# TankMermaid/GraphAligner

Hardware: AMD Instinct MI355X
Metric: aligned Gbp/sec (whole node), 10kb ONT reads vs chr-scale GFA (higher is better)
Workload: dtype u64

## Files before the change

__graft_entry__.py:

```python
import os
import subprocess
import sys

ROOT = os.path.dirname(os.path.abspath(__file__))
CSRC = os.path.join(ROOT, "graphaligner_amd", "csrc")
PRODUCT_SO = os.path.join(ROOT, "graphaligner_amd", "libgraphaligner_amd.so")
HIPCC = os.environ.get("HIPCC", "/opt/rocm/bin/hipcc")


def _run(cmd):
    print("+", " ".join(cmd), file=sys.stderr, flush=True)
    subprocess.check_call(cmd, stdout=sys.stderr)


def _stale(target, sources):
    if not os.path.exists(target):
        return True
    t = os.path.getmtime(target)
    return any(os.path.getmtime(s) > t for s in sources)


def build_stamped():
    obj = os.path.join(ROOT, "build")
    os.makedirs(obj, exist_ok=True)
# ... 11 lines not shown

def _hipcc_device(flags, out):
    import json
    import re
    cmd = [HIPCC, "--offload-arch=gfx950", "-O3", "-std=c++17", "-fPIC", "-Wno-unused-value", "-Rpass-analysis=kernel-resource-usage"] + flags + \
          ["-c", os.path.join(CSRC, "ga_device.hip"), "-o", out]
    print("+", " ".join(cmd), file=sys.stderr, flush=True)
    p = subprocess.run(cmd, stdout=subprocess.PIPE, stderr=subprocess.PIPE, text=True)
    table, cur = {}, None
    rest = []
    for line in p.stderr.splitlines():
        m = re.search(r"remark:\s+(.*?) \[-Rpass-analysis=kernel-resource-usage\]", line)
        if not m:
            rest.append(line)
            continue
        key, _, val = m.group(1).partition(":")
        key, val = key.strip(), val.strip()
        if key == "Function Name":
            name = subprocess.run(["c++filt", val], stdout=subprocess.PIPE, text=True).stdout.strip() or val
            name = re.sub(r"^void |\(anonymous namespace\)::|\(.*$", "", name)
            cur = table.setdefault(name, {})
        elif cur is not None:
            cur[key] = val
    sys.stderr.write("\n".join(l for l in rest if "warning" in l or "error" in l) + ("\n" if rest else ""))
    if p.returncode != 0:
        sys.stderr.write(p.stderr)
        raise subprocess.CalledProcessError(p.returncode, cmd)
    os.makedirs(os.path.dirname(RESOURCES_JSON), exist_ok=True)
    json.dump(table, open(RESOURCES_JSON, "w"), indent=1)
    print("%-52s %5s %5s %8s %7s %7s %5s %7s" % ("kernel", "VGPR", "AGPR", "scratch", "vSpill", "sSpill", "occ", "LDS"), file=sys.stderr)
    for name, r in table.items():
        print("%-52s %5s %5s %8s %7s %7s %5s %7s" % (name, r.get("VGPRs"), r.get("AGPRs"), r.get("ScratchSize [bytes/lane]"), r.get("VGPRs Spill"), r.get("SGPRs Spill"),
                                                     r.get("Occupancy [waves/SIMD]"), r.get("LDS Size [bytes/block]")), file=sys.stderr)
    no_scratch = ("ga_lanes_kernel", "ga_wide_kernel", "ga_wide_sparse_kernel", "ga_plan_", "ga_eq_words_", "ga_ops_", "ga_pileup_")
    bad = [n for n, r in table.items() if n.startswith(no_scratch) and int(r.get("ScratchSize [bytes/lane]", "0")) != 0]
    bad += [n for n, r in table.items() if n.startswith(("ga_lanes_kernel<10, 64>", "ga_plan_", "ga_eq_words_", "ga_ops_", "ga_pileup_")) and int(r.get("VGPRs Spill", "0")) != 0]
    if bad:
        raise RuntimeError("kernel resource check failed (private segment in a lanes = reads, state-in-HBM, plan or match-word kernel / vector "
                           "spills in <10,64>, a plan or a match-word kernel): %s" % ", ".join(bad))
    return table


def build_product(force=False):
    srcs = [os.path.join(CSRC, f) for f in os.listdir(CSRC)] + [os.path.join(ROOT, "include", "graphaligner_amd.h")]
    if not force and (os.environ.get("GA_SKIP_BUILD") == "1" or not _stale(PRODUCT_SO, srcs)) and os.path.exists(PRODUCT_SO):
        return
    obj = os.path.join(ROOT, "build")
    os.makedirs(obj, exist_ok=True)
    _run(["g++", "-std=c++17", "-O2", "-g", "-fPIC", "-ffp-contract=off", "-Wall", "-c", os.path.join(CSRC, "ga_host.cpp"), "-o", os.path.join(obj, "ga_host.o")])
    _run(["g++", "-std=c++17", "-O2", "-g", "-fPIC", "-Wall", "-c", os.path.join(CSRC, "ga_vgio.cpp"), "-o", os.path.join(obj, "ga_vgio.o")])
    _run(["g++", "-std=c++17", "-O2", "-g", "-fPIC", "-Wall", "-c", os.path.join(CSRC, "ga_seed_host.cpp"), "-o", os.path.join(obj, "ga_seed_host.o")])
    _hipcc_device(["-DGA_WAVES_EU=%s" % os.environ.get("GA_WAVES_EU", "6")], os.path.join(obj, "ga_device.o"))
    _run([HIPCC, "--offload-arch=gfx950", "-shared", "-pthread", "-o", PRODUCT_SO, os.path.join(obj, "ga_host.o"), os.path.join(obj, "ga_vgio.o"), os.path.join(obj, "ga_seed_host.o"), os.path.join(obj, "ga_device.o"), "-lz"])


def build():
    build_product()
    _run(["make", "-s", "-C", os.path.join(ROOT, "oracle")])
    _run(["make", "-s", "-C", os.path.join(ROOT, "tests", "emul")])
    _run(["make", "-s", "-C", os.path.join(ROOT, "tests", "emul"), "-f", "pileup.mk"])
    _run(["make", "-s", "-C", os.path.join(ROOT, "tests", "native")])
    sys.path.insert(0, ROOT)
    import graphaligner_amd
    from graphaligner_amd import binding
    binding.load()


# ... 21 lines not shown
```

graphaligner_amd/csrc/ga_device.hip:

```cpp
#include <hip/hip_runtime.h>

#include <algorithm>
#include <cstdio>
#include <cstdlib>
#include <cstring>
#include <memory>
#include <mutex>
#include <vector>

#include "../../include/graphaligner_amd.h"
#include "ga_backend.h"
#include "ga_kernel.h"
#include "ga_ladder.h"
#include "ga_lanes.h"
#include "ga_seed_dev.h"
#include "ga_plan.h"
#include "ga_ops.h"
#include "ga_pileup.h"

namespace {

#define HIP_OK(call) do { hipError_t e_ = (call); if (e_ != hipSuccess) { fprintf(stderr, "graphaligner_amd: %s failed: %s\n", #call, hipGetErrorString(e_)); return GA_E_DEVICE; } } while (0)

struct SlotLayout
// ... 77 lines not shown
		uint32_t job = L.job_list ? L.job_list[k] : k;
		gak::run_job<kWideNodes, true, false>(L, ws, slot, job);
		__syncthreads();
	}
}

__global__ void __launch_bounds__(64) ga_wide_sparse_kernel(GaLaunch L)
{
	const SlotLayout lay = slotLayout(L.cap_cols, L.max_slices, L.arena_words, L.trace_cap, L.sparse_bw, sizeof(gak::WaveState<kWideNodes>), kWideNodes);
	uint8_t* base = L.scratch + (uint64_t)blockIdx.x * L.slot_bytes;
	gak::WaveState<kWideNodes>& ws = *(gak::WaveState<kWideNodes>*)(base + lay.state);
	gak::Slot slot;
	slot.end_prev = (uint32_t*)(base + lay.endPrev);
	slot.end_cur = (uint32_t*)(base + lay.endCur);
	slot.slice_off = (uint32_t*)(base + lay.sliceOff);
	slot.arena = (uint32_t*)(base + lay.arena);
	slot.trace = base + lay.trace;
	slot.slice_flags = base + lay.flags;
	slot.ckpt = (uint32_t*)(base + lay.ckpt);
	slot.below_off = (uint32_t*)(base + lay.belowOff);
	slot.sparse = base + lay.sparse;
	slot.ovr = (uint32_t*)(base + lay.ovr);
	slot.sparse_max_bw = L.sparse_bw;
	while (true)
	{
		uint32_t k = gaw::wave_atomic_add(L.next_job, 1u);
		if (k >= L.n_jobs) break;
		uint32_t job = L.job_list ? L.job_list[k] : k;
		gak::run_job<kWideNodes, true, true>(L, ws, slot, job);
		__syncthreads();
	}
}

template <int N, int LW>
__global__ void __launch_bounds__(64) __attribute__((amdgpu_waves_per_eu(1, 2))) ga_lanes_kernel(gal::GaLanesLaunch L)
{
	using namespace gal;
	__shared__ uint32_t lds[Lay<N>::WORDS * LW + LW * kStageWords64 * 2 + 128];
	const int lane = (int)threadIdx.x;
	const WaveLayout lay = wave_layout<N>(L.cap_cols, L.cap_rows, L.max_slices, L.cap_moves, LW);
	uint8_t* base = L.scratch + (uint64_t)blockIdx.x * L.wave_bytes;
	while (true)
	{
		const uint32_t grp = gaw::wave_atomic_add(L.next_group, 1u);
		const uint64_t first = (uint64_t)grp * L.lanes_per_wave;
		if (first >= L.n_jobs) break;
		const bool hasJob = lane < (int)L.lanes_per_wave && lane < LW && first + (uint32_t)lane < L.n_jobs;
		const uint32_t jobIndex = hasJob ? (L.job_list ? L.job_list[first + (uint32_t)lane] : (uint32_t)(first + (uint32_t)lane)) : 0u;
		LaneMem m;
		m.lane = lane < LW ? lane : 0;
		m.tid = lane;
		m.flushPart = (uint32_t)lane % 12u; m.flushLane = (uint32_t)lane / 12u;
		m.ls = LW;
		m.lds.base = lds + (lane < LW ? lane : 0);
		m.lds.lw = LW;
		m.stage = (uint64_t*)(lds + Lay<N>::WORDS * LW);
		m.laneBlocks = lds + Lay<N>::WORDS * LW + LW * kStageWords64 * 2;
		m.usedChunks = 12u * (L.lanes_per_wave < (uint32_t)LW ? L.lanes_per_wave : (uint32_t)LW);
		m.endPrev = (uint32_t*)(base + lay.endA) + m.lane;
		m.endCur = (uint32_t*)(base + lay.endB) + m.lane;
		m.hdr = (uint32_t*)(base + lay.hdr) + m.lane;
		m.snodes = (uint32_t*)(base + lay.snodes) + m.lane;
		m.moves = (uint32_t*)(base + lay.moves) + m.lane;
		m.arena = base + lay.arena;
		LaneState st;
#if GA_STAMPS == 3
		const uint64_t wall0 = wall_clock64(), cyc0 = gaw::stamp();
#endif
		uint64_t tA = gaw::stamp(), tB, acc[4] = {0, 0, 0, 0};
#define GAL_LAP(i) do { tB = gaw::stamp(); acc[i] += tB - tA; tA = tB; } while (0)
		lane_begin<N>(L, m, st, jobIndex, hasJob);
		uint32_t blockTop = 0;
		for (uint32_t slice = 0; ; slice++)
		{
			lane_band<N>(L, m, st, slice);
			GAL_LAP(0);
			if (!__ballot(st.live)) break;
			fill_slice<N, 8, LW>(L.graph, m, st, slice, st.live, blockTop, L.cap_rows, L.cap_cols);
			GAL_LAP(1);
			lane_end_slice<N>(L, m, st, slice);
			GAL_LAP(2);
		}
		lane_finish<N>(L, m, st, hasJob);
		GAL_LAP(3);
#undef GAL_LAP
#ifdef GA_STAMPS
		if (hasJob && lane == 0) { GaJobOut* o = L.outs + st.job; o->stamps[1] = acc[0]; o->stamps[4] = acc[1]; o->stamps[0] = acc[2]; o->stamps[5] = acc[3]; o->stamps[2] = st.laps[0]; o->stamps[3] = st.laps[1]; o->stamps[6] = st.laps[2]; o->stamps[7] = st.laps[7];
#if GA_STAMPS == 4
			o->stamps[6] = acc[0]; o->stamps[7] = acc[1];
			for (int i = 0; i < 5; i++) o->stamps[i] = st.blaps[i];
#endif
#if GA_STAMPS == 3
			o->stamps[0] = wall0; o->stamps[1] = wall_clock64(); o->stamps[4] = gaw::stamp() - cyc0;
#endif
#if GA_STAMPS == 2
			o->stamps[0] = st.laps[4]; o->stamps[1] = st.laps[5]; o->stamps[4] = st.laps[6];
#endif
		}
#endif
		__syncthreads();
	}
}

__device__ __forceinline__ void eq_words_body(const uint8_t* __restrict__ seq, const GaEqFill* __restrict__ fills, uint32_t nFills, const uint8_t* __restrict__ lut,
                                              uint32_t padCode, uint64_t* __restrict__ eq, uint8_t* __restrict__ flags, uint8_t* __restrict__ rows)
{
	__shared__ uint8_t t[512];
	const uint32_t lane = threadIdx.x;
	for (uint32_t i = lane; i < 512; i += 64) t[i] = lut[i];
	__syncthreads();
	for (uint32_t fi = blockIdx.x; fi < nFills; fi += gridDim.x)
	{
		const GaEqFill f = fills[fi];
		const uint8_t* s = seq + f.seq_off;
		bool bad = false;
		for (uint32_t r0 = 0; r0 < f.padded; r0 += 64)
		{
			const uint32_t k = r0 + lane;
			uint32_t code = padCode;
			if (k < f.n) code = f.backward ? t[256 + s[f.n - 1 - k]] : t[s[f.pos + k]];
			rows[f.eq_slice * 64 + k] = (uint8_t)code;
			const uint64_t e0 = __ballot(code & 1u), e1 = __ballot(code & 2u), e2 = __ballot(code & 4u), e3 = __ballot(code & 8u);
			const uint64_t inv = __ballot(code & GA_ROW_INVALID);
			const uint32_t last = (uint32_t)__builtin_amdgcn_readlane((int)code, 63);
			const uint64_t meta = (uint64_t)((last >> 4) & 7u) | (inv ? 8u : 0u);
			if (lane < 5) eq[(f.eq_slice + r0 / 64) * 5 + lane] = lane == 0 ? e0 : lane == 1 ? e1 : lane == 2 ? e2 : lane == 3 ? e3 : meta;
			bad = bad || inv != 0;
		}
		if (lane == 0) flags[fi] = bad ? 1 : 0;
	}
}
__global__ void __launch_bounds__(64) ga_eq_words_kernel(const uint8_t* __restrict__ seq, const GaEqFill* __restrict__ fills, uint32_t nFills, const uint8_t* __restrict__ lut,
                                                         uint32_t padCode, uint64_t* __restrict__ eq, uint8_t* __restrict__ flags, uint8_t* __restrict__ rows)
{
// ... 604 lines not shown
		uint32_t maxRows = 0;
		for (uint32_t i : list) maxRows = std::max(maxRows, jobs[i].n_rows);
		P.max_slices = std::max<uint32_t>(maxRows / 64, 1);
		P.cap_cols = std::min<uint32_t>(N * 256u, 0xff00u);
		P.cap_moves = maxRows * 2 + 1024;
		const uint32_t ldsBytes = gal::Lay<N>::WORDS * LW * 4 + LW * gal::kStageWords64 * 8 + 512;
		const uint32_t wavesPerCu = std::max<uint32_t>(1, std::min<uint32_t>(8, 163840u / ldsBytes));
		auto layoutFor = [&](uint32_t lanes) {
			P.cap_rows = (uint32_t)std::min<uint64_t>(((uint64_t)P.max_slices * rowsPerSlice * lanes + 64 + 7u) & ~7ull, 0x7ffffff0ull);
			return gal::wave_layout<N>(P.cap_cols, P.cap_rows, P.max_slices, P.cap_moves, LW);
		};
		gal::WaveLayout lay = layoutFor(LW);
		const uint64_t fit = scratchBudget() / std::max<uint64_t>(lay.bytes, 1);
		uint64_t slotsHere = std::max<uint64_t>(1, std::min<uint64_t>((uint64_t)g->cus * wavesPerCu, std::max<uint64_t>(fit, 64)));
		if (knobs.waveSlots) slotsHere = std::min<uint64_t>(slotsHere, knobs.waveSlots);
		uint32_t lanesPer = LW;
		if (knobs.spread > 1) lanesPer = (uint32_t)std::min<int>(LW, knobs.spread);
		else if (knobs.spread && list.size() * 10 < slotsHere * LW * 6)
			lanesPer = (uint32_t)std::min<uint64_t>(LW, std::max<uint64_t>(8, (list.size() + slotsHere - 1) / slotsHere));
		P.lanes_per_wave = lanesPer;
		lay = layoutFor(lanesPer);
		P.wave_bytes = lay.bytes;
		const uint64_t groups = (list.size() + lanesPer - 1) / lanesPer;
		const uint32_t waves = (uint32_t)std::max<uint64_t>(1, std::min<uint64_t>(slotsHere, groups));
		bool fromPool = false;
		uint8_t* scratch = takeScratch((size_t)waves * lay.bytes, fromPool);
		if (!scratch) return 0;
		P.scratch = scratch;
		int rc = uploadList(list);
		if (!rc)
		{
			hipMemsetAsync(L.next_job, 0, 16, stream);
			hipEventRecord(evA, stream);
			hipLaunchKernelGGL((ga_lanes_kernel<N, LW>), dim3(waves), dim3(64), 0, stream, P);
			float ms = 0;
			rc = afterPass(ms);
			if (first) { st.main_ms = ms; st.main_variant = N * 1000 + 80 + (LW == 64 ? 0 : 1); st.slots = waves; st.waves_per_cu = wavesPerCu; st.scratch_bytes = (uint64_t)waves * lay.bytes; }
			if (knobs.debugPasses) fprintf(stderr, "graphaligner_amd: lanes pass <%d,%d>: %zu jobs on %u waves of %u lanes (%.1f GB scratch), %.2f ms\n", N, LW, list.size(), waves, lanesPer, waves * (double)lay.bytes / 1e9, ms);
#if GA_STAMPS == 3
			{
				uint64_t lo = ~0ull, hi = 0, n = 0; double life = 0, cyc = 0, lateStart = 0;
				for (auto& o : outs) if (o.stamps[1]) { lo = std::min(lo, o.stamps[0]); hi = std::max(hi, o.stamps[1]); }
				for (auto& o : outs) if (o.stamps[1]) { n++; life += (double)(o.stamps[1] - o.stamps[0]); cyc += (double)o.stamps[4]; lateStart = std::max(lateStart, (double)(o.stamps[0] - lo)); }
				{
					std::vector<std::pair<double, uint64_t>> lives;
					for (auto& o : outs) if (o.stamps[1]) lives.push_back({(double)(o.stamps[1] - o.stamps[0]) / 1e5, o.stamps[7]});
					std::sort(lives.begin(), lives.end());
					auto at = [&](double q) { return lives[(size_t)(q * (lives.size() - 1))]; };
					if (!lives.empty()) fprintf(stderr, "graphaligner_amd: wave life ms p10 %.2f p50 %.2f p90 %.2f p99 %.2f max %.2f; traceback rounds of the p10 / p50 / p99 / max wave: %llu / %llu / %llu / %llu, fast iterations %llu / %llu / %llu / %llu\n",
						at(0.1).first, at(0.5).first, at(0.9).first, at(0.99).first, at(1.0).first,
						(unsigned long long)(at(0.1).second & 0xffffffffu), (unsigned long long)(at(0.5).second & 0xffffffffu), (unsigned long long)(at(0.99).second & 0xffffffffu), (unsigned long long)(at(1.0).second & 0xffffffffu),
						(unsigned long long)(at(0.1).second >> 32), (unsigned long long)(at(0.5).second >> 32), (unsigned long long)(at(0.99).second >> 32), (unsigned long long)(at(1.0).second >> 32));
				}
				if (n) fprintf(stderr, "graphaligner_amd: %llu waves: first start to last end %.3f ms, mean wave life %.3f ms = %.1f M shader cycles (%.2f GHz), latest start %.3f ms after the first\n",
				               (unsigned long long)n, (hi - lo) / 1e5, life / n / 1e5, cyc / n / 1e6, cyc / life / 10.0, lateStart / 1e5);
			}
#endif
		}
		if (fromPool) g->givePool();
		return rc;
	}

	struct WaveKernel
	{
		void (*kernel)(GaLaunch);
		int maxN;
		bool general;
// ... 404 lines not shown
```

graphaligner_amd/csrc/ga_lanes.h:

```cpp
#pragma once
#include <stdint.h>

#include "ga_types.h"

namespace gal {

#ifdef GA_EMULATE
#define GAL_FN inline
#else
#define GAL_FN __device__ __forceinline__
#endif

#if defined(GA_STAMPS) && !defined(GA_EMULATE)
GAL_FN uint64_t lap_clock() { return __builtin_readcyclecounter(); }
#else
GAL_FN uint64_t lap_clock() { return 0; }
#endif

constexpr int W = 64;
constexpr int INF = 0x3fffffff;
constexpr uint32_t kCutoff = 200000;
constexpr int kRecBytes = 24;
constexpr int kHdrWords = 8;
constexpr uint32_t kNone = 0xffu;
// ... 1035 lines not shown
	{
		const unsigned long long prev = atomicCAS((unsigned long long*)top, seen, seen + (unsigned long long)bytes);
		if (prev == seen) return seen;
		seen = prev;
	}
	return ~0ull;
}
GAL_FN bool claim_for_wave(uint64_t* top, uint64_t cap, uint64_t bytes, uint64_t& at)
{
	const uint64_t active = __ballot(1);
	const int lane = (int)(threadIdx.x & 63);
	uint64_t before = 0, total = 0;
	for (uint64_t m = active; m; m &= m - 1)
	{
		const int src = __builtin_ctzll(m);
		const uint64_t b = ((uint64_t)(uint32_t)__shfl((int)(uint32_t)(bytes >> 32), src, 64) << 32) | (uint32_t)__shfl((int)(uint32_t)bytes, src, 64);
		if (src < lane) before += b;
		total += b;
	}
	const int leader = __builtin_ctzll(active);
	uint64_t base = ~0ull;
	if (lane == leader) base = claim_cas(top, cap, total);
	base = ((uint64_t)(uint32_t)__shfl((int)(uint32_t)(base >> 32), leader, 64) << 32) | (uint32_t)__shfl((int)(uint32_t)base, leader, 64);
	if (base != ~0ull) { at = base + before; return true; }
	bool ok = false;
	for (uint64_t m = active; m; m &= m - 1)
	{
		if (lane == __builtin_ctzll(m)) { const uint64_t a = claim_cas(top, cap, bytes); if (a != ~0ull) { at = a; ok = true; } }
	}
	return ok;
}
#endif

template <int N> GAL_FN void lane_finish(const GaLanesLaunch& L, const LaneMem& m, LaneState& st, bool hasJob)
{
	typedef Lay<N> LY;
	if (!hasJob) return;
	const GaDevGraph& g = L.graph;
	const Lds& l = m.lds;
	GaJobOut out;
	out.status = st.status; out.score = 0x7fffffff; out.n_valid = 0; out.n_run = st.nRun; out.trace_len = 0; out.max_band_nodes = st.maxBandNodes;
	out.n_columns = st.nColumns; out.trace_off = 0; out.start_node = 0; out.start_offset = 0; out.start_row = 0; out.reserved2 = 0;
	out.n_node_steps = 0; out.reserved3 = 0;
	for (int i = 0; i < 8; i++) out.stamps[i] = 0;
	int status = st.status;
	uint32_t kept = st.nPushed;
	if (status == GA_OK && kept > 0)
	{
		bool ok = (m.hdr[((uint64_t)(kept - 1) * kHdrWords + 5) * m.ls] & 1u) != 0;
		while (!ok)
		{
			kept--;
			if (kept == 0) break;
			ok = (m.hdr[((uint64_t)(kept - 1) * kHdrWords + 5) * m.ls] & 2u) != 0;
		}
	}
	out.n_valid = status == GA_OK ? kept : 0;
	uint32_t len = 0, nodeSteps = 0;
	if (status == GA_OK && kept > 0)
	{
		const int big = (int)st.nRows;
		uint32_t sIdx = kept - 1;
		uint32_t nN = 0, pN = 0, curRow = 0, prvRow = 0;
		uint32_t aN = 0, aRow = 0;
		int tCN = LY::T_CN, tCB = LY::T_CB, tPN = LY::T_PN, tPB = LY::T_PB;
		auto loadHeader = [&](uint32_t sl, uint32_t& count, uint32_t& rowBase) {
			const uint32_t* h = m.hdr + (uint64_t)sl * kHdrWords * m.ls;
			count = h[0];
			rowBase = h[6 * m.ls];
// ... 3 lines not shown
			for (uint32_t k = 0; k < count; k += 4)
			{
				uint32_t a[8];
#pragma unroll
				for (int i = 0; i < 8; i++) a[i] = sn[(uint64_t)(2 * k + (uint32_t)i) * m.ls];
#pragma unroll
				for (int i = 0; i < 4; i++) if (k + (uint32_t)i < count) { l.wr(tn + (int)k + i, a[2 * i]); l.wr(tb + (int)k + i, a[2 * i + 1]); }
			}
		};
		auto loadTableFrom = [&](int tn, int tb, uint32_t sl, uint32_t count, uint32_t from) {
			const uint32_t* sn = m.snodes + (uint64_t)sl * 2 * N * m.ls;
			for (uint32_t k = from; k < count; k++) { const uint32_t a0 = sn[(uint64_t)(2 * k) * m.ls], a1 = sn[(uint64_t)(2 * k + 1) * m.ls]; l.wr(tn + (int)k, a0); l.wr(tb + (int)k, a1); }
		};
		struct NodeRec { uint64_t firstCol; uint32_t inDeg; uint32_t nb[4], nbLen[4]; };
		auto loadRec = [&](uint32_t n, NodeRec& nr) {
			const uint32_t* rec = g_rec(g, n);
			nr.firstCol = ((uint64_t)rec[1] << 32) | rec[0];
			nr.inDeg = rec[3] & 0xffffu;
#pragma unroll
			for (int k = 0; k < 4; k++) { nr.nb[k] = rec[8 + k]; nr.nbLen[k] = rec[12 + k]; }
		};
		loadHeader(sIdx, nN, curRow);
		if (sIdx > 0) loadHeader(sIdx - 1, pN, prvRow);
		if (sIdx > 1) loadHeader(sIdx - 2, aN, aRow);
		loadTable(tCN, tCB, sIdx, nN);
		if (sIdx > 0) loadTable(tPN, tPB, sIdx - 1, pN);
		const uint32_t* h = m.hdr + (uint64_t)sIdx * kHdrWords * m.ls;
		out.score = (int32_t)h[2 * m.ls];
		uint32_t node = l.rd(tCN + (int)h[3 * m.ls]);
		int offset = (int)h[4 * m.ls];
		uint32_t row = sIdx * W + (W - 1);
		out.start_node = node; out.start_offset = (uint32_t)offset; out.start_row = row;
		bool tracing = true;
		const bool emitRuns = L.emit_runs != 0;
		const uint32_t traceRows = st.traceRows;
		const uint32_t capRunWords = (L.cap_moves + 3) / 4 + 8;
		uint32_t nRuns = 0, runLastOff = (uint32_t)offset, runLastRow = row;
		bool started = row < traceRows;
		auto emitRun = [&](uint32_t n, uint32_t firstOff, uint32_t firstRow) {
			if (5 * (nRuns + 1) > capRunWords) { status = GA_CAP_TRACE; tracing = false; return; }
			uint32_t* d = m.moves + (uint64_t)(5 * nRuns) * m.ls;
			d[0] = n; d[1 * m.ls] = firstOff; d[2 * m.ls] = firstRow; d[3 * m.ls] = runLastOff; d[4 * m.ls] = runLastRow;
			nRuns++;
		};
		uint64_t e[4];
		auto loadEq = [&](uint32_t sl) { const uint64_t* q = st.eq + (uint64_t)sl * 5; e[0] = q[0]; e[1] = q[1]; e[2] = q[2]; e[3] = q[3]; };
		loadEq(sIdx);
		auto recordIn = [&](int tn, int tb, uint32_t count, uint32_t rowBase, uint32_t n, uint32_t off, Col& c) -> bool {
			const int sl = find_in(l, tn, (int)count, n);
			c.vp = 0; c.vn = 0; c.before = 0;
			if (sl < 0) return false;
			rec_load_col<8>(m, rowBase + l.rd(tb + sl) + off, c);
			return true;
		};
		uint32_t pack = 0;
#ifdef GA_DEBUG_SITE
		uint32_t site = 0;
#define GAL_SITE(n) site = (n)
#else
#define GAL_SITE(n)
#endif
		constexpr int kWin = Lay<N>::T_WINCOLS;
		constexpr int tWIN = Lay<N>::T_WIN;
#ifndef GAL_BURST_SLACK
#define GAL_BURST_SLACK 4
#endif
		constexpr int kBurst = kWin - GAL_BURST_SLACK;
		Col q0, q1;
		q0.vp = q0.vn = 0; q0.before = 0; q1 = q0;
		bool needSetup = true;
		uint32_t slotRow = 0, recNode = 0xffffffffu, inDeg = 0;
		uint32_t nb[4] = {0, 0, 0, 0}, nbLen[4] = {0, 0, 0, 0};
		uint64_t firstCol = 0;
		NodeRec nx = NodeRec();
		uint32_t nxNode = 0xffffffffu, nxSlotRow = 0;
		uint64_t wbases = 0;
		int wLo = 1, wHi = 0;
		bool crossed = false, xStarted = false;
		uint32_t xRowBefore = 0, xRowAfter = 0;
		uint32_t capMoves = L.cap_moves;
		uint32_t roundsLeft = 2 * L.cap_moves + 4096;
#ifndef GA_EMULATE
		asm volatile("" : "+v"(capMoves));
#endif
		auto winRead = [&](int o, Col& c) {
			const int at = tWIN + (o - wLo) * 5;
			c.vp = ((uint64_t)l.rd(at + 1) << 32) | l.rd(at);
			c.vn = ((uint64_t)l.rd(at + 3) << 32) | l.rd(at + 2);
			c.before = (int)l.rd(at + 4);
		};
		auto putMove = [&](int res, int via) {
			if (emitRuns) return;
			const uint32_t code = res == 1 ? GA_MOVE_LEFT : res == 2 ? GA_MOVE_DIAG : GA_MOVE_UP;
			pack |= (code | (res == 3 ? 0u : ((uint32_t)via << 2))) << (8 * (len & 3));
			if ((len & 3) == 3) { m.moves[(uint64_t)(len >> 2) * m.ls] = pack; pack = 0; }
			len++;
		};
		auto bases32 = [&](uint64_t col, uint32_t w0, uint32_t w1, uint32_t w2) -> uint64_t {
			const uint32_t sh = 2 * (uint32_t)(col & 15);
			return (((uint64_t)w0 | ((uint64_t)w1 << 32)) >> sh) | (sh ? (uint64_t)w2 << (64 - sh) : 0ull);
		};
#ifdef GA_EMULATE
#define GAL_ANY(x) (x)
#else
#define GAL_ANY(x) (__ballot(x) != 0)
#endif
		bool firstRound = true;
		uint64_t lapT = lap_clock();
		while (GAL_ANY(tracing))
		{
			const bool first = firstRound;
			firstRound = false;
			{ const uint64_t t2 = lap_clock(); st.laps[1] += t2 - lapT; lapT = t2; }
			if (!first)
			{
				int r = (int)(row - sIdx * W);
				uint64_t mR = r < 0 ? 0ull : r < 63 ? ~(~0ull << (r + 1)) : ~0ull;
				int here = q0.before + __builtin_popcountll(q0.vp & mR) - __builtin_popcountll(q0.vn & mR);
				Col q2;
				winRead(((offset >= wLo + 2) & (offset <= wHi)) ? offset - 2 : wLo, q2);
				for (int it = 0; it < kBurst; it++)
				{
					const bool fast = tracing & (r > 0) & (offset > wLo) & (offset <= wHi) & (len + 8 < capMoves);
					if (!GAL_ANY(fast)) break;
#ifdef GA_STAMPS
					st.laps[7] += 1ull << 32;
#endif
					const int sr = r & 63;
					const int horizontal = q1.before + __builtin_popcountll(q1.vp & mR) - __builtin_popcountll(q1.vn & mR);
					const int diagonal = horizontal - (int)((uint32_t)(q1.vp >> sr) & 1u) + (int)((uint32_t)(q1.vn >> sr) & 1u);
					const int up = here - (int)((uint32_t)(q0.vp >> sr) & 1u) + (int)((uint32_t)(q0.vn >> sr) & 1u);
					const int base = (int)(wbases >> (2 * ((offset - wLo) & 31))) & 3;
					const int want = here - 1 + (int)((e[base] >> sr) & 1);
					const bool left = horizontal == here - 1;
					const bool diag = !left & (diagonal == want);
					const bool bad = (horizontal < here - 1) | (!left & (diagonal < want)) | (!left & !diag & (up != here - 1));
					const bool ok = fast & !bad;
					status = fast & bad ? GA_ASSERTION : status;
#ifdef GA_DEBUG_SITE
					site = fast & bad ? ((horizontal < here - 1) ? 1 : (!left & (diagonal < want)) ? 2 : 3) : site;
#endif
					tracing = tracing & !(fast & bad);
					const bool colMove = ok & (left | diag), rowMove = ok & !left;
					const bool crossNow = colMove & (offset == 0);
					xRowBefore = crossNow ? row : xRowBefore;
					xStarted = crossNow ? started : xStarted;
					crossed = crossed | crossNow;
					here = ok ? (left ? horizontal : diag ? diagonal : up) : here;
					row -= rowMove ? 1u : 0u;
					r -= rowMove ? 1 : 0;
					mR = rowMove ? mR >> 1 : mR;
					xRowAfter = crossNow ? row : xRowAfter;
					offset -= colMove ? 1 : 0;
					q0.vp = colMove ? q1.vp : q0.vp; q0.vn = colMove ? q1.vn : q0.vn; q0.before = colMove ? q1.before : q0.before;
					q1.vp = colMove ? q2.vp : q1.vp; q1.vn = colMove ? q2.vn : q1.vn; q1.before = colMove ? q2.before : q1.before;
					winRead(((offset >= wLo + 2) & (offset <= wHi)) ? offset - 2 : wLo, q2);
					if (emitRuns)
					{
						const bool begin = ok & !started & (row < traceRows);
						runLastOff = begin ? (uint32_t)offset : runLastOff;
						runLastRow = begin ? row : runLastRow;
						started = started | begin;
					}
					else if (ok) putMove(left ? 1 : diag ? 2 : 3, 0);
				}
			}
			{ const uint64_t t2 = lap_clock(); st.laps[0] += t2 - lapT; lapT = t2; }
#ifdef GA_STAMPS
			st.laps[7] += 1;
#endif
			if (tracing)
			{
				const uint64_t g0 = lap_clock();
				if (row == 0xffffffffu) { tracing = false; continue; }
				if (len + 8 >= capMoves) { status = GA_CAP_TRACE; tracing = false; continue; }
				if (roundsLeft-- == 0) { status = GA_PUNT; tracing = false; continue; }
				const uint32_t safeRow = 0;
				if (crossed)
				{
					const uint32_t oldNode = node, L0 = nbLen[0];
					node = nb[0]; offset += (int)L0; wLo += (int)L0; wHi += (int)L0;
					nodeSteps++;
					slotRow = nxSlotRow;
					firstCol = nx.firstCol; inDeg = nx.inDeg;
#pragma unroll
					for (int k = 0; k < 4; k++) { nb[k] = nx.nb[k]; nbLen[k] = nx.nbLen[k]; }
					recNode = node;
					crossed = false;
					if (emitRuns)
					{
						if (xStarted) { emitRun(oldNode, 0, xRowBefore); runLastOff = L0 - 1; runLastRow = xRowAfter; }
						else if (started) runLastOff += L0;
					}
				}
				if (!tracing) continue;
				if (inDeg > 4) { status = GA_PUNT; tracing = false; continue; }
				const int r = (int)(row - sIdx * W);
				const bool chained = !first && inDeg == 1 && nb[0] != node && nxNode == nb[0];
				const bool decision = !first && !(r > 0 && (offset > 0 || (chained && find_in(l, tCN, (int)nN, nb[0]) >= 0)));
				bool changed = false;
				NodeRec spec = NodeRec();
				uint32_t specNode = 0xffffffffu;
				if (GAL_ANY(decision))
				{
				if (decision)
				{
				const bool needWin = !(offset >= wLo && offset <= wHi && (offset == 0 || offset > wLo));
				const bool atStart = offset == 0;
				const bool atTop = r == 0 && sIdx > 0;
				Col wc[kWin];
				uint32_t sq0 = 0, sq1 = 0, sq2 = 0;
				const int nLoA = offset >= kWin - 1 ? offset - (kWin - 1) : 0;
				{
#pragma unroll
					for (int i = 0; i < kWin; i++) rec_load_col<8>(m, needWin && nLoA + i <= offset ? slotRow + (uint32_t)(nLoA + i) : safeRow, wc[i]);
					const uint64_t col = needWin ? firstCol + (uint64_t)nLoA : 0ull;
					const uint32_t* q = g.seq2 + (col >> 4);
					sq0 = q[0]; sq1 = q[1]; sq2 = q[2];
				}
				Col nc[4];
#pragma unroll
				for (int k = 0; k < 4; k++) { nc[k].vp = nc[k].vn = 0; nc[k].before = 0; }
				bool nIn[4] = {false, false, false, false};
				{
					uint32_t nbRow[4];
#pragma unroll
// ... 17 lines not shown
				{
					uint32_t rowA = safeRow, rowU = safeRow;
					if (atTop)
					{
						const int slU = find_in(l, tPN, (int)pN, node);
						if (slU >= 0) { uIn = true; rowU = prvRow + l.rd(tPB + slU) + (uint32_t)offset; }
						if (offset > 0) { aIn = uIn; rowA = uIn ? rowU - 1 : safeRow; }
						else if (inDeg > 0)
						{
							const int slA = find_in(l, tPN, (int)pN, nb[0]);
							if (slA >= 0) { aIn = true; rowA = prvRow + l.rd(tPB + slA) + nbLen[0] - 1; }
						}
					}
					rec_load_col<8>(m, rowA, ca);
					rec_load_col<8>(m, rowU, cu);
				}
				if (needWin)
				{
					wLo = nLoA; wHi = offset;
					wbases = bases32(firstCol + (uint64_t)wLo, sq0, sq1, sq2);
#pragma unroll
					for (int i = 0; i < kWin; i++)
					{
						if (wLo + i <= wHi)
						{
							const int at = tWIN + i * 5;
							l.wr(at, (uint32_t)wc[i].vp); l.wr(at + 1, (uint32_t)(wc[i].vp >> 32)); l.wr(at + 2, (uint32_t)wc[i].vn); l.wr(at + 3, (uint32_t)(wc[i].vn >> 32)); l.wr(at + 4, (uint32_t)wc[i].before);
						}
					}
					winRead(offset, q0);
					if (offset > wLo) winRead(offset - 1, q1);
				}
				const int here = col_value(q0.vp, q0.vn, q0.before, r);
				if (emitRuns && !started && row < traceRows) { started = true; runLastOff = (uint32_t)offset; runLastRow = row; }
				if (row == 0 && node == st.seedNode && (here == 0 || here == 1))
				{
					if (emitRuns && started) emitRun(node, (uint32_t)offset, row);
					row = 0xffffffffu; tracing = false; continue;
				}
				const uint32_t rowBefore = row;
				const int base = (int)(wbases >> (2 * (offset - wLo))) & 3;
				const bool match = ((e[base] >> r) & 1) != 0;
				int res = 0, via = 0;
				const uint32_t curNode = node, curOffset = (uint32_t)offset;
				auto decide = [&](int horizontal, int diagonal, uint32_t un, uint32_t uo) -> int {
					if (horizontal < here - 1) return -1;
					if (horizontal == here - 1) { node = un; offset = (int)uo; return 1; }
					if (match)
					{
						if (diagonal < here) return -1;
						if (diagonal == here) { node = un; offset = (int)uo; row = row - 1; return 2; }
					}
					else
					{
						if (diagonal < here - 1) return -1;
						if (diagonal == here - 1) { node = un; offset = (int)uo; row = row - 1; return 2; }
					}
					return 0;
				};
				auto aboveOf = [&](bool in, const Col& c, uint32_t n) -> int {
					if (sIdx == 0) return n == st.seedNode ? 0 : big;
					return in ? col_value(c.vp, c.vn, c.before, W - 1) : big;
				};
				auto valueAbove = [&](uint32_t n, uint32_t o) -> int {
					if (sIdx == 0) return n == st.seedNode ? 0 : big;
					Col c;
					if (!recordIn(tPN, tPB, pN, prvRow, n, o, c)) return big;
					return col_value(c.vp, c.vn, c.before, W - 1);
				};
				if (curOffset == 0)
				{
#pragma unroll
					for (int k = 0; k < 4; k++)
					{
						if ((uint32_t)k < inDeg && res == 0)
						{
							const uint32_t mo = nbLen[k] - 1;
							via = k;
							const int horizontal = nIn[k] ? col_value(nc[k].vp, nc[k].vn, nc[k].before, r) : big;
							int diagonal = 0;
							if (horizontal > here - 1) diagonal = r > 0 ? (nIn[k] ? col_value(nc[k].vp, nc[k].vn, nc[k].before, r - 1) : big) : k == 0 ? aboveOf(aIn, ca, nb[0]) : valueAbove(nb[k], mo);
							res = decide(horizontal, diagonal, nb[k], mo);
						}
					}
					if (res == 1 || res == 2) { needSetup = true; nodeSteps++; }
				}
				else
				{
					const int horizontal = col_value(q1.vp, q1.vn, q1.before, r);
					int diagonal = 0;
					if (horizontal > here - 1) diagonal = r > 0 ? col_value(q1.vp, q1.vn, q1.before, r - 1) : aboveOf(aIn, ca, curNode);
					res = decide(horizontal, diagonal, curNode, curOffset - 1);
				}
				if (res < 0) { GAL_SITE(5); status = GA_ASSERTION; tracing = false; continue; }
				if (res == 0)
				{
					const int up = r > 0 ? col_value(q0.vp, q0.vn, q0.before, r - 1) : aboveOf(uIn, cu, curNode);
					if (up != here - 1) { GAL_SITE(6); status = GA_ASSERTION; tracing = false; continue; }
					row = row - 1;
					res = 3;
				}
				if (row == 0xffffffffu)
				{
					if (emitRuns && started) emitRun(curNode, curOffset, rowBefore);
					tracing = false; continue;
				}
				putMove(res, via);
				if (emitRuns)
				{
					if (curOffset == 0 && res != 3 && node != curNode)
					{
						if (started) { emitRun(curNode, curOffset, rowBefore); if (!tracing) continue; }
						runLastOff = (uint32_t)offset; runLastRow = row;
					}
					if (!started && row < traceRows) { started = true; runLastOff = (uint32_t)offset; runLastRow = row; }
				}
				changed = res >= 2 && r == 0;
				if (changed)
				{
					sIdx--;
					int t = tCN; tCN = tPN; tPN = t;
					t = tCB; tCB = tPB; tPB = t;
					nN = pN; curRow = prvRow;
					pN = aN; prvRow = aRow;
					needSetup = true;
				}
				}
				}
				const uint64_t g1 = lap_clock();
				if (needSetup)
				{
					const int slot = find_in(l, tCN, (int)nN, node);
					if (slot < 0) { GAL_SITE(4); status = GA_ASSERTION; tracing = false; continue; }
					slotRow = curRow + l.rd(tCB + slot);
					wLo = 1; wHi = 0;
				}
				if (node != recNode && node == specNode)
				{
					firstCol = spec.firstCol; inDeg = spec.inDeg;
#pragma unroll
					for (int k = 0; k < 4; k++) { nb[k] = spec.nb[k]; nbLen[k] = spec.nbLen[k]; }
// ... 74 lines not shown
				{
					const uint64_t col = refill && needRec ? firstCol + (uint64_t)xLo : 0ull;
					const uint32_t* q = g.seq2 + (col >> 4);
					const uint32_t t0 = q[0], t1 = q[1], t2 = q[2];
					if (refill && needRec) { sq0 = t0; sq1 = t1; sq2 = t2; }
				}
				if (refill)
				{
					wLo = nLo; wHi = offset;
					const uint64_t bx = bases32(firstCol + (uint64_t)xLo, sq0, sq1, sq2);
					const int ny = xLo - nLo;
					wbases = ny > 0 ? ((bases32(colY, sy0, sy1, sy2) & ~(~0ull << (2 * ny))) | (bx << (2 * ny))) : bx;
#pragma unroll
					for (int i = 0; i < kWin; i++)
					{
						if (wLo + i <= wHi)
						{
							const int at = tWIN + i * 5;
							l.wr(at, (uint32_t)wd[i].vp); l.wr(at + 1, (uint32_t)(wd[i].vp >> 32)); l.wr(at + 2, (uint32_t)wd[i].vn); l.wr(at + 3, (uint32_t)(wd[i].vn >> 32)); l.wr(at + 4, (uint32_t)wd[i].before);
						}
					}
				}
				winRead(offset, q0);
				if (offset > wLo) winRead(offset - 1, q1);
				{ const uint64_t g3 = lap_clock(); st.laps[4] += g1 - g0; st.laps[5] += g2 - g1; st.laps[6] += g3 - g2; }
			}
		}
#undef GAL_ANY
#undef GAL_SITE
#ifdef GA_DEBUG_SITE
		if (status != GA_OK) out.stamps[site & 7] = 1;
#endif
		{ const uint64_t t2 = lap_clock(); st.laps[1] += t2 - lapT; lapT = t2; }
		if (!emitRuns && (len & 3)) m.moves[(uint64_t)(len >> 2) * m.ls] = pack;
		st.laps[3] = lap_clock();
		if (status == GA_OK)
		{
			const uint32_t words = emitRuns ? 5 * nRuns : (len + 3) / 4;
			uint64_t at = 0;
			bool claimed = false;
#ifdef GA_EMULATE
			if (*L.trace_top + (uint64_t)words * 4 <= L.trace_pool_cap) { at = *L.trace_top; *L.trace_top += (uint64_t)words * 4; claimed = true; }
#else
			claimed = claim_for_wave(L.trace_top, L.trace_pool_cap, (uint64_t)words * 4, at);
#endif
			if (!claimed) status = GA_CAP_TRACE;
			else
			{
				uint32_t* dst = (uint32_t*)(L.traces + at);
				for (uint32_t k = 0; k < words; k += 8)
				{
					uint32_t a[8];
#pragma unroll
					for (int i = 0; i < 8; i++) a[i] = m.moves[(uint64_t)(k + (uint32_t)i) * m.ls];
#pragma unroll
					for (int i = 0; i < 8; i++) if (k + (uint32_t)i < words) dst[k + (uint32_t)i] = a[i];
				}
				out.trace_off = at;
				out.trace_len = emitRuns ? nRuns : len;
				out.reserved3 = emitRuns ? 1u : 0u;
				out.n_node_steps = nodeSteps;
			}
		}
	}
	{ const uint64_t t2 = lap_clock(); st.laps[2] += t2 - st.laps[3]; }
	out.status = status;
	if (status != GA_OK) { out.n_valid = 0; out.score = 0x7fffffff; out.trace_len = 0; }
	L.outs[st.job] = out;
}

}
```

Baseline: 15.36.

## Specialize lanes traceback kernel per output form and streamline fast burst loop

Splits the lanes kernel into two compile-time variants, one emitting node runs and one emitting packed moves, chosen at launch from emit_runs. Code for the unused form is removed at compile time. The traceback fast burst loop is reworked: the window read uses a precomputed LDS pointer stride, bounds checks fold into one unsigned compare, and the per-iteration started/crossed bookkeeping is hoisted out of the loop. This cuts ALU work and register pressure in the hot traceback path, at the cost of a second kernel instantiation and more subtle state logic that could diverge from the original semantics.

```diff
diff --git a/__graft_entry__.py b/__graft_entry__.py
--- a/__graft_entry__.py
+++ b/__graft_entry__.py
@@ -67,7 +67,7 @@
     for name, r in table.items():
         print("%-52s %5s %5s %8s %7s %7s %5s %7s" % (name, r.get("VGPRs"), r.get("AGPRs"), r.get("ScratchSize [bytes/lane]"), r.get("VGPRs Spill"), r.get("SGPRs Spill"),
                                                      r.get("Occupancy [waves/SIMD]"), r.get("LDS Size [bytes/block]")), file=sys.stderr)
-    no_scratch = ("ga_lanes_kernel", "ga_wide_kernel", "ga_wide_sparse_kernel", "ga_plan_", "ga_eq_words_", "ga_ops_", "ga_pileup_")
+    no_scratch = ("ga_lanes_kernel", "ga_lanes_moves_kernel", "ga_wide_kernel", "ga_wide_sparse_kernel", "ga_plan_", "ga_eq_words_", "ga_ops_", "ga_pileup_")
     bad = [n for n, r in table.items() if n.startswith(no_scratch) and int(r.get("ScratchSize [bytes/lane]", "0")) != 0]
     bad += [n for n, r in table.items() if n.startswith(("ga_lanes_kernel<10, 64>", "ga_plan_", "ga_eq_words_", "ga_ops_", "ga_pileup_")) and int(r.get("VGPRs Spill", "0")) != 0]
     if bad:
diff --git a/graphaligner_amd/csrc/ga_device.hip b/graphaligner_amd/csrc/ga_device.hip
--- a/graphaligner_amd/csrc/ga_device.hip
+++ b/graphaligner_amd/csrc/ga_device.hip
@@ -133,11 +133,11 @@
 	}
 }
 
-template <int N, int LW>
-__global__ void __launch_bounds__(64) __attribute__((amdgpu_waves_per_eu(1, 2))) ga_lanes_kernel(gal::GaLanesLaunch L)
+template <int N> constexpr int kLanesLdsWords(int lw) { return gal::Lay<N>::WORDS * lw + lw * gal::kStageWords64 * 2 + 128; }
+template <int N, int LW, int FORM>
+__device__ __forceinline__ void lanes_wave(const gal::GaLanesLaunch& L, uint32_t* lds)
 {
 	using namespace gal;
-	__shared__ uint32_t lds[Lay<N>::WORDS * LW + LW * kStageWords64 * 2 + 128];
 	const int lane = (int)threadIdx.x;
 	const WaveLayout lay = wave_layout<N>(L.cap_cols, L.cap_rows, L.max_slices, L.cap_moves, LW);
 	uint8_t* base = L.scratch + (uint64_t)blockIdx.x * L.wave_bytes;
@@ -182,7 +182,7 @@
 			lane_end_slice<N>(L, m, st, slice);
 			GAL_LAP(2);
 		}
-		lane_finish<N>(L, m, st, hasJob);
+		lane_finish<N, FORM>(L, m, st, hasJob);
 		GAL_LAP(3);
 #undef GAL_LAP
 #ifdef GA_STAMPS
@@ -201,6 +201,18 @@
 #endif
 		__syncthreads();
 	}
+}
+template <int N, int LW>
+__global__ void __launch_bounds__(64) __attribute__((amdgpu_waves_per_eu(1, 2))) ga_lanes_kernel(gal::GaLanesLaunch L)
+{
+	__shared__ uint32_t lds[kLanesLdsWords<N>(LW)];
+	lanes_wave<N, LW, 1>(L, lds);
+}
+template <int N, int LW>
+__global__ void __launch_bounds__(64) __attribute__((amdgpu_waves_per_eu(1, 2))) ga_lanes_moves_kernel(gal::GaLanesLaunch L)
+{
+	__shared__ uint32_t lds[kLanesLdsWords<N>(LW)];
+	lanes_wave<N, LW, 0>(L, lds);
 }
 
 __device__ __forceinline__ void eq_words_body(const uint8_t* __restrict__ seq, const GaEqFill* __restrict__ fills, uint32_t nFills, const uint8_t* __restrict__ lut,
@@ -871,7 +883,8 @@
 		{
 			hipMemsetAsync(L.next_job, 0, 16, stream);
 			hipEventRecord(evA, stream);
-			hipLaunchKernelGGL((ga_lanes_kernel<N, LW>), dim3(waves), dim3(64), 0, stream, P);
+			if (P.emit_runs) hipLaunchKernelGGL((ga_lanes_kernel<N, LW>), dim3(waves), dim3(64), 0, stream, P);
+			else hipLaunchKernelGGL((ga_lanes_moves_kernel<N, LW>), dim3(waves), dim3(64), 0, stream, P);
 			float ms = 0;
 			rc = afterPass(ms);
 			if (first) { st.main_ms = ms; st.main_variant = N * 1000 + 80 + (LW == 64 ? 0 : 1); st.slots = waves; st.waves_per_cu = wavesPerCu; st.scratch_bytes = (uint64_t)waves * lay.bytes; }
diff --git a/graphaligner_amd/csrc/ga_lanes.h b/graphaligner_amd/csrc/ga_lanes.h
--- a/graphaligner_amd/csrc/ga_lanes.h
+++ b/graphaligner_amd/csrc/ga_lanes.h
@@ -1091,9 +1091,11 @@
 }
 #endif
 
-template <int N> GAL_FN void lane_finish(const GaLanesLaunch& L, const LaneMem& m, LaneState& st, bool hasJob)
+template <int N, int FORM = -1> GAL_FN void lane_finish(const GaLanesLaunch& L, const LaneMem& m, LaneState& st, bool hasJob)
 {
 	typedef Lay<N> LY;
+	static_assert(FORM >= -1 && FORM <= 1, "output form: -1 at run time, 0 moves, 1 node runs");
+	constexpr bool kMayRun = FORM != 0, kMayMove = FORM != 1;
 	if (!hasJob) return;
 	const GaDevGraph& g = L.graph;
 	const Lds& l = m.lds;
@@ -1163,16 +1165,19 @@
 		uint32_t row = sIdx * W + (W - 1);
 		out.start_node = node; out.start_offset = (uint32_t)offset; out.start_row = row;
 		bool tracing = true;
-		const bool emitRuns = L.emit_runs != 0;
+		const bool emitRuns = FORM < 0 ? L.emit_runs != 0 : FORM != 0;
 		const uint32_t traceRows = st.traceRows;
 		const uint32_t capRunWords = (L.cap_moves + 3) / 4 + 8;
 		uint32_t nRuns = 0, runLastOff = (uint32_t)offset, runLastRow = row;
 		bool started = row < traceRows;
 		auto emitRun = [&](uint32_t n, uint32_t firstOff, uint32_t firstRow) {
-			if (5 * (nRuns + 1) > capRunWords) { status = GA_CAP_TRACE; tracing = false; return; }
-			uint32_t* d = m.moves + (uint64_t)(5 * nRuns) * m.ls;
-			d[0] = n; d[1 * m.ls] = firstOff; d[2 * m.ls] = firstRow; d[3 * m.ls] = runLastOff; d[4 * m.ls] = runLastRow;
-			nRuns++;
+			if constexpr (kMayRun)
+			{
+				if (5 * (nRuns + 1) > capRunWords) { status = GA_CAP_TRACE; tracing = false; return; }
+				uint32_t* d = m.moves + (uint64_t)(5 * nRuns) * m.ls;
+				d[0] = n; d[1 * m.ls] = firstOff; d[2 * m.ls] = firstRow; d[3 * m.ls] = runLastOff; d[4 * m.ls] = runLastRow;
+				nRuns++;
+			}
 		};
 		uint64_t e[4];
 		auto loadEq = [&](uint32_t sl) { const uint64_t* q = st.eq + (uint64_t)sl * 5; e[0] = q[0]; e[1] = q[1]; e[2] = q[2]; e[3] = q[3]; };
@@ -1220,12 +1225,21 @@
 			c.vn = ((uint64_t)l.rd(at + 3) << 32) | l.rd(at + 2);
 			c.before = (int)l.rd(at + 4);
 		};
+		auto winReadAt = [&](int w, Col& c) {
+			const uint32_t* p = l.base + w;
+			c.vp = ((uint64_t)p[l.lw] << 32) | p[0];
+			c.vn = ((uint64_t)p[3 * l.lw] << 32) | p[2 * l.lw];
+			c.before = (int)p[4 * l.lw];
+		};
 		auto putMove = [&](int res, int via) {
-			if (emitRuns) return;
-			const uint32_t code = res == 1 ? GA_MOVE_LEFT : res == 2 ? GA_MOVE_DIAG : GA_MOVE_UP;
-			pack |= (code | (res == 3 ? 0u : ((uint32_t)via << 2))) << (8 * (len & 3));
-			if ((len & 3) == 3) { m.moves[(uint64_t)(len >> 2) * m.ls] = pack; pack = 0; }
-			len++;
+			if constexpr (kMayMove)
+			{
+				if (emitRuns) return;
+				const uint32_t code = res == 1 ? GA_MOVE_LEFT : res == 2 ? GA_MOVE_DIAG : GA_MOVE_UP;
+				pack |= (code | (res == 3 ? 0u : ((uint32_t)via << 2))) << (8 * (len & 3));
+				if ((len & 3) == 3) { m.moves[(uint64_t)(len >> 2) * m.ls] = pack; pack = 0; }
+				len++;
+			}
 		};
 		auto bases32 = [&](uint64_t col, uint32_t w0, uint32_t w1, uint32_t w2) -> uint64_t {
 			const uint32_t sh = 2 * (uint32_t)(col & 15);
@@ -1234,7 +1248,7 @@
 #ifdef GA_EMULATE
 #define GAL_ANY(x) (x)
 #else
-#define GAL_ANY(x) (__ballot(x) != 0)
+#define GAL_ANY(x) (__builtin_amdgcn_ballot_w64((bool)(x)) != 0)
 #endif
 		bool firstRound = true;
 		uint64_t lapT = lap_clock();
@@ -1248,12 +1262,21 @@
 				int r = (int)(row - sIdx * W);
 				uint64_t mR = r < 0 ? 0ull : r < 63 ? ~(~0ull << (r + 1)) : ~0ull;
 				int here = q0.before + __builtin_popcountll(q0.vp & mR) - __builtin_popcountll(q0.vn & mR);
+				const int colStride = 5 * l.lw, w0 = tWIN * l.lw;
+				const int span = wHi - wLo, wLo1 = wLo + 1, rel0 = offset - wLo;
+				uint32_t spanT = (tracing & (span > 0)) ? (uint32_t)span : 0u;
+				int w2 = ((rel0 >= 1) & (rel0 <= span)) ? w0 + (rel0 - 2) * colStride : w0;
+				const bool startedIn = started;
+				const uint32_t beginRow = startedIn ? 0xfffffffeu : traceRows - 1;
+				(void)beginRow;
 				Col q2;
-				winRead(((offset >= wLo + 2) & (offset <= wHi)) ? offset - 2 : wLo, q2);
-				for (int it = 0; it < kBurst; it++)
-				{
-					const bool fast = tracing & (r > 0) & (offset > wLo) & (offset <= wHi) & (len + 8 < capMoves);
-					if (!GAL_ANY(fast)) break;
+				winReadAt(w2, q2);
+				for (int it = 0; ; it++)
+				{
+					const uint32_t u = (uint32_t)(offset - wLo1);
+					bool fast = (r > 0) & (u < spanT);
+					if constexpr (kMayMove) fast = fast & (len + 8 < capMoves);
+					if ((it >= kBurst) | !GAL_ANY(fast)) break;
 #ifdef GA_STAMPS
 					st.laps[7] += 1ull << 32;
 #endif
@@ -1261,7 +1284,7 @@
 					const int horizontal = q1.before + __builtin_popcountll(q1.vp & mR) - __builtin_popcountll(q1.vn & mR);
 					const int diagonal = horizontal - (int)((uint32_t)(q1.vp >> sr) & 1u) + (int)((uint32_t)(q1.vn >> sr) & 1u);
 					const int up = here - (int)((uint32_t)(q0.vp >> sr) & 1u) + (int)((uint32_t)(q0.vn >> sr) & 1u);
-					const int base = (int)(wbases >> (2 * ((offset - wLo) & 31))) & 3;
+					const int base = (int)(wbases >> ((2 * u + 2) & 62)) & 3;
 					const int want = here - 1 + (int)((e[base] >> sr) & 1);
 					const bool left = horizontal == here - 1;
 					const bool diag = !left & (diagonal == want);
@@ -1271,29 +1294,45 @@
 #ifdef GA_DEBUG_SITE
 					site = fast & bad ? ((horizontal < here - 1) ? 1 : (!left & (diagonal < want)) ? 2 : 3) : site;
 #endif
-					tracing = tracing & !(fast & bad);
+					spanT = (fast & bad) ? 0u : spanT;
 					const bool colMove = ok & (left | diag), rowMove = ok & !left;
-					const bool crossNow = colMove & (offset == 0);
-					xRowBefore = crossNow ? row : xRowBefore;
-					xStarted = crossNow ? started : xStarted;
-					crossed = crossed | crossNow;
+					bool crossNow = false;
+					if constexpr (kMayRun) { crossNow = colMove & (offset == 0); xRowBefore = crossNow ? row : xRowBefore; }
 					here = ok ? (left ? horizontal : diag ? diagonal : up) : here;
 					row -= rowMove ? 1u : 0u;
 					r -= rowMove ? 1 : 0;
 					mR = rowMove ? mR >> 1 : mR;
-					xRowAfter = crossNow ? row : xRowAfter;
+					if constexpr (kMayRun) xRowAfter = crossNow ? row : xRowAfter;
 					offset -= colMove ? 1 : 0;
+					w2 -= colMove ? colStride : 0;
 					q0.vp = colMove ? q1.vp : q0.vp; q0.vn = colMove ? q1.vn : q0.vn; q0.before = colMove ? q1.before : q0.before;
 					q1.vp = colMove ? q2.vp : q1.vp; q1.vn = colMove ? q2.vn : q1.vn; q1.before = colMove ? q2.before : q1.before;
-					winRead(((offset >= wLo + 2) & (offset <= wHi)) ? offset - 2 : wLo, q2);
-					if (emitRuns)
+					winReadAt(w2, q2);
+					if constexpr (kMayRun)
 					{
-						const bool begin = ok & !started & (row < traceRows);
+						const bool begin = rowMove & (row == beginRow);
 						runLastOff = begin ? (uint32_t)offset : runLastOff;
 						runLastRow = begin ? row : runLastRow;
-						started = started | begin;
 					}
-					else if (ok) putMove(left ? 1 : diag ? 2 : 3, 0);
+					if constexpr (kMayMove)
+					{
+						if (!emitRuns)
+						{
+							const uint32_t code = left ? GA_MOVE_LEFT : diag ? GA_MOVE_DIAG : GA_MOVE_UP;
+							pack |= ok ? code << (8 * (len & 3)) : 0u;
+							const bool full = ok & ((len & 3) == 3);
+							if (full) m.moves[(uint64_t)(len >> 2) * m.ls] = pack;
+							pack = full ? 0u : pack;
+							len += ok ? 1u : 0u;
+						}
+					}
+				}
+				tracing = tracing & (status == GA_OK);
+				crossed = offset < 0;
+				if constexpr (kMayRun)
+				{
+					xStarted = startedIn | (xRowBefore < traceRows);
+					started = startedIn | (row < traceRows);
 				}
 			}
 			{ const uint64_t t2 = lap_clock(); st.laps[0] += t2 - lapT; lapT = t2; }
@@ -1304,7 +1343,7 @@
 			{
 				const uint64_t g0 = lap_clock();
 				if (row == 0xffffffffu) { tracing = false; continue; }
-				if (len + 8 >= capMoves) { status = GA_CAP_TRACE; tracing = false; continue; }
+				if constexpr (kMayMove) { if (len + 8 >= capMoves) { status = GA_CAP_TRACE; tracing = false; continue; } }
 				if (roundsLeft-- == 0) { status = GA_PUNT; tracing = false; continue; }
 				const uint32_t safeRow = 0;
 				if (crossed)
@@ -1318,11 +1357,15 @@
 					for (int k = 0; k < 4; k++) { nb[k] = nx.nb[k]; nbLen[k] = nx.nbLen[k]; }
 					recNode = node;
 					crossed = false;
-					if (emitRuns)
+					if constexpr (kMayRun)
 					{
-						if (xStarted) { emitRun(oldNode, 0, xRowBefore); runLastOff = L0 - 1; runLastRow = xRowAfter; }
-						else if (started) runLastOff += L0;
+						if (emitRuns)
+						{
+							if (xStarted) { emitRun(oldNode, 0, xRowBefore); runLastOff = L0 - 1; runLastRow = xRowAfter; }
+							else if (started) runLastOff += L0;
+						}
 					}
+					(void)oldNode;
 				}
 				if (!tracing) continue;
 				if (inDeg > 4) { status = GA_PUNT; tracing = false; continue; }
@@ -1406,10 +1449,10 @@
 					if (offset > wLo) winRead(offset - 1, q1);
 				}
 				const int here = col_value(q0.vp, q0.vn, q0.before, r);
-				if (emitRuns && !started && row < traceRows) { started = true; runLastOff = (uint32_t)offset; runLastRow = row; }
+				if constexpr (kMayRun) { if (emitRuns && !started && row < traceRows) { started = true; runLastOff = (uint32_t)offset; runLastRow = row; } }
 				if (row == 0 && node == st.seedNode && (here == 0 || here == 1))
 				{
-					if (emitRuns && started) emitRun(node, (uint32_t)offset, row);
+					if constexpr (kMayRun) { if (emitRuns && started) emitRun(node, (uint32_t)offset, row); }
 					row = 0xffffffffu; tracing = false; continue;
 				}
 				const uint32_t rowBefore = row;
@@ -1476,11 +1519,11 @@
 				}
 				if (row == 0xffffffffu)
 				{
-					if (emitRuns && started) emitRun(curNode, curOffset, rowBefore);
+					if constexpr (kMayRun) { if (emitRuns && started) emitRun(curNode, curOffset, rowBefore); }
 					tracing = false; continue;
 				}
 				putMove(res, via);
-				if (emitRuns)
+				if constexpr (kMayRun) if (emitRuns)
 				{
 					if (curOffset == 0 && res != 3 && node != curNode)
 					{
@@ -1621,11 +1664,14 @@
 		if (status != GA_OK) out.stamps[site & 7] = 1;
 #endif
 		{ const uint64_t t2 = lap_clock(); st.laps[1] += t2 - lapT; lapT = t2; }
-		if (!emitRuns && (len & 3)) m.moves[(uint64_t)(len >> 2) * m.ls] = pack;
+		if constexpr (kMayMove) { if (!emitRuns && (len & 3)) m.moves[(uint64_t)(len >> 2) * m.ls] = pack; }
 		st.laps[3] = lap_clock();
 		if (status == GA_OK)
 		{
-			const uint32_t words = emitRuns ? 5 * nRuns : (len + 3) / 4;
+			uint32_t words = 0;
+			if constexpr (FORM == 1) words = 5 * nRuns;
+			else if constexpr (FORM == 0) words = (len + 3) / 4;
+			else words = emitRuns ? 5 * nRuns : (len + 3) / 4;
 			uint64_t at = 0;
 			bool claimed = false;
 #ifdef GA_EMULATE
@@ -1646,8 +1692,9 @@
 					for (int i = 0; i < 8; i++) if (k + (uint32_t)i < words) dst[k + (uint32_t)i] = a[i];
 				}
 				out.trace_off = at;
-				out.trace_len = emitRuns ? nRuns : len;
-				out.reserved3 = emitRuns ? 1u : 0u;
+				if constexpr (FORM == 1) { out.trace_len = nRuns; out.reserved3 = 1u; }
+				else if constexpr (FORM == 0) { out.trace_len = len; out.reserved3 = 0u; }
+				else { out.trace_len = emitRuns ? nRuns : len; out.reserved3 = emitRuns ? 1u : 0u; }
 				out.n_node_steps = nodeSteps;
 			}
 		}
```

New measurement: 16.24, median of 6. 1.06x the previous value.
